# wzjin2017/fhe-fed

Hardware: AMD Instinct MI355X
Metric: ciphertexts aggregated/sec (+ encode+enc / dec+decode ms), N clients, ring 2^15 L=4 (higher is better)
Workload: dtype u64; 1 GPU; cfg3: 16 learners/GPU x ResNet-18 (11689512 params -> 714 cts of 16384 slots), ring 2^15, L=4 towers; ring_dim=32768, towers=4, learners_total=16, cts_per_learner=714, parallelism=dp1 (one GPU, no collective), layout=arena

## Files before the change

fhe-fed_amd/csrc/dev_common.h:

```cpp
#pragma once

#include <hip/hip_runtime.h>

#include "shelfi_internal.h"

namespace shelfi {

typedef uint32_t u32x4 __attribute__((ext_vector_type(4)));

__device__ __forceinline__ uint64_t addmod(uint64_t a, uint64_t b, uint64_t q) {
  uint64_t s = a + b;
  return s >= q ? s - q : s;
}
__device__ __forceinline__ uint64_t submod(uint64_t a, uint64_t b, uint64_t q) {
  return a >= b ? a - b : a + q - b;
}
__device__ __forceinline__ uint64_t shoup_mul(uint64_t x, uint64_t w, uint64_t wp, uint64_t q) {
  uint64_t hi = __umul64hi(x, wp);
  uint64_t r = x * w - hi * q;
  return r >= q ? r - q : r;
}
__device__ __forceinline__ uint64_t red64(uint64_t x, uint64_t q, uint64_t one_sh) {
  uint64_t hi = __umul64hi(x, one_sh);
  uint64_t r = x - hi * q;
// ... 11 lines not shown
  const uint32_t c1 = x1 * w0 + x0 * w1, c2 = h1 * n0 + h0 * n1;
  uint32_t hi;
  asm("v_add3_u32 %0, %1, %2, %3" : "=v"(hi) : "v"((uint32_t)(lo >> 32)), "v"(c1), "v"(c2));
  return ((uint64_t)hi << 32) | (uint32_t)lo;
}
__device__ __forceinline__ uint64_t shoup_lazy_add(uint64_t x, uint64_t w, uint64_t wp, uint64_t q, uint64_t a) {
  const uint64_t h = umulhi_approx(x, wp), nq = (uint64_t)0 - q;
  const uint32_t x0 = (uint32_t)x, x1 = (uint32_t)(x >> 32), w0 = (uint32_t)w, w1 = (uint32_t)(w >> 32);
  const uint32_t h0 = (uint32_t)h, h1 = (uint32_t)(h >> 32), n0 = (uint32_t)nq, n1 = (uint32_t)(nq >> 32);
  const uint64_t lo = (uint64_t)h0 * n0 + ((uint64_t)x0 * w0 + a);
  const uint32_t c1 = x1 * w0 + x0 * w1, c2 = h1 * n0 + h0 * n1;
  uint32_t hi;
  asm("v_add3_u32 %0, %1, %2, %3" : "=v"(hi) : "v"((uint32_t)(lo >> 32)), "v"(c1), "v"(c2));
  return ((uint64_t)hi << 32) | (uint32_t)lo;
}
__device__ __forceinline__ uint64_t shoup_lazy_sub(uint64_t x, uint64_t w, uint64_t wp, uint64_t q) {
  return x * w - umulhi_approx(x, wp) * q;
}
__device__ __forceinline__ uint64_t sub4q_if_ge(uint64_t X, uint64_t q) {
  uint64_t d;
  const bool borrow = __builtin_sub_overflow(X, q << 2, &d);
  return borrow ? X : d;
}
__device__ __forceinline__ void ct_bfly(uint64_t& X, uint64_t& Y, uint64_t W, uint64_t Wp,
                                        uint64_t q) {
  const uint64_t x = sub4q_if_ge(X, q);
  const uint64_t t = shoup_lazy(Y, W, Wp, q);
  X = x + t;
  Y = x + (q << 2) - t;
}
__device__ __forceinline__ void gs_bfly(uint64_t& X, uint64_t& Y, uint64_t W, uint64_t Wp,
                                        uint64_t q) {
  const uint64_t s = X + Y;
  const uint64_t d = X + (q << 2) - Y;
  X = sub4q_if_ge(s, q);
  Y = shoup_lazy_sub(d, W, Wp, q);
}
__device__ __forceinline__ uint32_t bfi32(uint32_t m, uint32_t a, uint32_t b) {
  uint32_t r;
  asm("v_bfi_b32 %0, %1, %2, %3" : "=v"(r) : "v"(m), "v"(a), "v"(b));
  return r;
}
__device__ __forceinline__ uint64_t csub_neg(uint64_t x, uint64_t negc) {
  const uint64_t d = x + negc;
  const uint32_t m = (uint32_t)((int32_t)(uint32_t)(d >> 32) >> 31);
  const uint32_t lo = bfi32(m, (uint32_t)x, (uint32_t)d);
  const uint32_t hi = bfi32(m, (uint32_t)(x >> 32), (uint32_t)(d >> 32));
  return ((uint64_t)hi << 32) | lo;
}
__device__ __forceinline__ uint64_t red_any(uint64_t x, const TowerConst& c) {
  const uint32_t k = __umulhi((uint32_t)(x >> 32), c.red_r) >> c.red_sh;
  const uint64_t r = x + (uint64_t)k * (uint32_t)c.nq + ((uint64_t)(k * (uint32_t)(c.nq >> 32)) << 32);
  return csub_neg(r, c.nq);
}
constexpr uint64_t kNoRedQ = 1ull << 57;
constexpr bool fwd_red_at(int s) {
  int B = 1;
  for (int i = 0; i < s; ++i) B = (B + 4 > 16 ? 8 : B) + 4;
  return B + 4 > 16;
}
constexpr int fwd_bound(int S) {
  int B = 1;
  for (int i = 0; i < S; ++i) B = (B + 4 > 16 ? 8 : B) + 4;
  return B;
}
template <bool RED>
__device__ __forceinline__ void ct_bfly_s(uint64_t& X, uint64_t& Y, uint64_t W, uint64_t Wp,
                                          uint64_t q, uint64_t n8q) {
  const uint64_t x = RED ? csub_neg(X, n8q) : X;
  const uint64_t s = shoup_lazy_add(Y, W, Wp, q, x);
  Y = (x << 1) + (q << 2) - s;
  X = s;
}

__device__ __forceinline__ void gs_bfly_s(uint64_t& X, uint64_t& Y, uint64_t W, uint64_t Wp,
                                          uint64_t q, uint64_t n4q) {
  const uint64_t x = X, y = Y;
  X = csub_neg(x + y, n4q);
  Y = shoup_lazy(x + (q << 2) - y, W, Wp, q);
}
template <bool B8>
__device__ __forceinline__ void gs_bfly_b(uint64_t& X, uint64_t& Y, uint64_t W, uint64_t Wp, uint64_t q,
                                          uint64_t n8q) {
  const uint64_t x = X, y = Y;
  X = B8 ? csub_neg(x + y, n8q) : x + y;
  Y = shoup_lazy(x + (q << (B8 ? 3 : 2)) - y, W, Wp, q);
}
template <bool IN8>
__device__ constexpr bool gs_in8(int v, int a) {
  return v == 0 ? IN8 : ((a >> (v - 1)) & 1) == 0;
}
__device__ __forceinline__ uint64_t canon8(uint64_t x, uint64_t q) {
  x = x >= 4 * q ? x - 4 * q : x;
  x = x >= 2 * q ? x - 2 * q : x;
  return x >= q ? x - q : x;
}
__device__ __forceinline__ uint64_t canon4(uint64_t x, uint64_t q) {
  x = x >= 2 * q ? x - 2 * q : x;
  return x >= q ? x - q : x;
}

__device__ __forceinline__ uint64_t mulmod_generic(uint64_t a, uint64_t b, const TowerConst& c) {
  uint64_t hi = __umul64hi(a, b), lo = a * b;
  return addmod(shoup_mul(hi, c.r64, c.r64_shoup, c.q), red64(lo, c.q, c.one_shoup), c.q);
}
__device__ __forceinline__ uint64_t mod_signed_dev(int64_t v, const TowerConst& c) {
// ... 425 lines not shown
```

fhe-fed_amd/csrc/keyswitch.hip:

```cpp
#include <hip/hip_runtime.h>

#include <algorithm>

#include "dev_common.h"
#include "shelfi_internal.h"

namespace shelfi {

typedef unsigned __int128 du128;

#define NTT_DISPATCH_KS(LOGRV, KERNEL, ...)                                               \
  switch (LOGRV) {                                                                       \
    case 1: hipLaunchKernelGGL(KERNEL<1>, __VA_ARGS__); break;                           \
    case 2: hipLaunchKernelGGL(KERNEL<2>, __VA_ARGS__); break;                           \
    case 3: hipLaunchKernelGGL(KERNEL<3>, __VA_ARGS__); break;                           \
    case 4: hipLaunchKernelGGL(KERNEL<4>, __VA_ARGS__); break;                           \
    case 5: hipLaunchKernelGGL(KERNEL<5>, __VA_ARGS__); break;                           \
    case 6: hipLaunchKernelGGL(KERNEL<6>, __VA_ARGS__); break;                           \
    default: throw Error{SHELFI_ERR_ARG, "EvalMult: unsupported ring dimension"};        \
  }

__device__ __forceinline__ uint64_t red128(du128 acc, const TowerConst& c) {
  const uint64_t hi = (uint64_t)(acc >> 64), lo = (uint64_t)acc;
  return addmod(shoup_mul(hi, c.r64, c.r64_shoup, c.q), red64(lo, c.q, c.one_shoup), c.q);
}
__device__ __forceinline__ du128 mul128(uint64_t a, uint64_t b) { return (du128)a * b; }

__device__ __forceinline__ void digit_span(const KsArgs& a, uint32_t j, uint32_t& s, uint32_t& cnt) {
  s = j * a.alpha;
  cnt = min(a.alpha, a.Ll - s);
}
__device__ __forceinline__ uint64_t ext_base(const KsArgs& a, uint32_t j, uint64_t K) {
  uint64_t base = 0;
  for (uint32_t i = 0; i < j; ++i) {
    uint32_t s, cnt;
    digit_span(a, i, s, cnt);
    base += (uint64_t)(a.T - cnt) * K;
  }
  return base << a.logN;
}

__global__ __launch_bounds__(256) void ks_tensor_intt_kernel(const uint64_t* x, const uint64_t* y, uint32_t Ll,
                                                             uint32_t logN, uint32_t blkLog,
                                                             const uint64_t* __restrict__ itw,
                                                             const uint64_t* __restrict__ itwp,
                                                             const TowerConst* __restrict__ tq, uint64_t* out,
                                                             uint64_t* __restrict__ d2e,
                                                             uint64_t* __restrict__ d2c) {
  extern __shared__ __attribute__((aligned(16))) uint64_t sm[];
  const uint32_t N = 1u << logN, blk = 1u << blkLog, sh = logN - blkLog;
  const uint64_t row = blockIdx.x >> sh;
  const uint32_t b = blockIdx.x & ((1u << sh) - 1);
  const uint64_t k = row / Ll;
  const uint32_t t = (uint32_t)(row % Ll);
  const TowerConst c = tq[t];
  const uint64_t q = c.q;
  const uint64_t off = ((uint64_t)t << logN) + ((uint64_t)b << blkLog);
  const uint64_t i0 = ((k * 2 * Ll) << logN) + off, i1 = (((k * 2 + 1) * Ll) << logN) + off;
  const uint64_t id = (row << logN) + ((uint64_t)b << blkLog);
  const ulonglong2* A0 = reinterpret_cast<const ulonglong2*>(x + i0);
  const ulonglong2* A1 = reinterpret_cast<const ulonglong2*>(x + i1);
  const ulonglong2* B0 = reinterpret_cast<const ulonglong2*>(y + i0);
  const ulonglong2* B1 = reinterpret_cast<const ulonglong2*>(y + i1);
  ulonglong2* O0 = reinterpret_cast<ulonglong2*>(out + i0);
  ulonglong2* O1 = reinterpret_cast<ulonglong2*>(out + i1);
  ulonglong2* E2 = reinterpret_cast<ulonglong2*>(d2e + id);
  for (uint32_t p = threadIdx.x; p < blk / 2; p += 256) {
    const ulonglong2 a0 = A0[p], a1 = A1[p], b0 = B0[p], b1 = B1[p];
    const ulonglong2 r0 = make_ulonglong2(mulmod_generic(a0.x, b0.x, c), mulmod_generic(a0.y, b0.y, c));
    const ulonglong2 r1 =
        make_ulonglong2(addmod(mulmod_generic(a0.x, b1.x, c), mulmod_generic(a1.x, b0.x, c), q),
                        addmod(mulmod_generic(a0.y, b1.y, c), mulmod_generic(a1.y, b0.y, c), q));
    const ulonglong2 r2 = make_ulonglong2(mulmod_generic(a1.x, b1.x, c), mulmod_generic(a1.y, b1.y, c));
    O0[p] = r0;
    O1[p] = r1;
    E2[p] = r2;
    lds_put2(sm, p, r2);
  }
  __syncthreads();
  ks_intt_block_out(sm, blkLog, b, logN, itw + (uint64_t)t * N, itwp + (uint64_t)t * N, c, d2c + id);
}

__global__ __launch_bounds__(256) void modup_kernel(const uint64_t* __restrict__ c, uint64_t K,
                                                    KsArgs a, uint64_t* __restrict__ ext) {
  const uint32_t N = 1u << a.logN, bpr = N >> 8;
  const uint64_t row = blockIdx.x / bpr;
  const uint32_t n = (blockIdx.x % bpr) * 256 + threadIdx.x;
  const uint32_t j = (uint32_t)(row / K);
  const uint64_t k = row % K;
  uint32_t s, cnt;
  digit_span(a, j, s, cnt);
  uint64_t yv[kMaxTowers];
  for (uint32_t i = 0; i < cnt; ++i) {
    const TowerConst ci = a.tq[s + i];
    yv[i] = shoup_mul(c[((k * a.Ll + s + i) << a.logN) + n], a.mu_inv[j * a.alpha + i],
                      a.mu_inv_sh[j * a.alpha + i], ci.q);
  }
  const uint32_t Tf = a.T - cnt;
  uint64_t* __restrict__ o = ext + ext_base(a, j, K) + ((k * Tf) << a.logN) + n;
  for (uint32_t u = 0; u < Tf; ++u) {
    const uint32_t t = u < s ? u : u + cnt;
    du128 acc = 0;
    const uint64_t* __restrict__ h = a.mu_hat + (uint64_t)j * a.alpha * a.T + t;
    for (uint32_t i = 0; i < cnt; ++i) acc += mul128(yv[i], h[(uint64_t)i * a.T]);
    o[(uint64_t)u << a.logN] = red128(acc, a.te[t]);
  }
}

template <int LOGR>
__global__ __launch_bounds__(256) void modup_cols_kernel(const uint64_t* __restrict__ c, uint64_t K, KsArgs a,
                                                         const uint64_t* __restrict__ tw,
                                                         const uint64_t* __restrict__ twp,
                                                         uint64_t* __restrict__ ext) {
  constexpr int R = 1 << LOGR;
  const uint32_t N = 1u << a.logN, BLK = N >> LOGR, bpp = BLK / 256;
  const uint64_t row = blockIdx.x / bpp;
  const uint32_t col = (blockIdx.x % bpp) * 256 + threadIdx.x;
  const uint32_t j = (uint32_t)(row / K);
  const uint64_t k = row % K;
  uint32_t s, cnt;
  digit_span(a, j, s, cnt);
  uint64_t y[2][R];
#pragma unroll
  for (int i = 0; i < 2; ++i) {
    if ((uint32_t)i < cnt) {
      const TowerConst ci = a.tq[s + i];
      const uint64_t w = a.mu_inv[j * a.alpha + i], wp = a.mu_inv_sh[j * a.alpha + i];
      const uint64_t* __restrict__ src = c + ((k * a.Ll + s + i) << a.logN) + col;
#pragma unroll
      for (int r = 0; r < R; ++r) y[i][r] = shoup_mul(src[(uint64_t)r * BLK], w, wp, ci.q);
    }
  }
  const uint32_t Tf = a.T - cnt;
  uint64_t* __restrict__ o = ext + ext_base(a, j, K) + ((k * Tf) << a.logN) + col;
  for (uint32_t u = 0; u < Tf; ++u) {
    const uint32_t t = u < s ? u : u + cnt;
    const TowerConst ct = a.te[t];
    const uint64_t h0 = a.mu_hat[(uint64_t)j * a.alpha * a.T + t];
    const uint64_t h1 = cnt > 1 ? a.mu_hat[((uint64_t)j * a.alpha + 1) * a.T + t] : 0;
    uint64_t x[R];
#pragma unroll
    for (int r = 0; r < R; ++r) {
      du128 acc = mul128(y[0][r], h0);
      if (cnt > 1) acc += mul128(y[1][r], h1);
      x[r] = red128(acc, ct);
    }
    const uint64_t* __restrict__ w = tw + (uint64_t)t * N;
    const uint64_t* __restrict__ wp = twp + (uint64_t)t * N;
#pragma unroll
    for (int st = 0; st < LOGR; ++st) {
      const int m = 1 << st, tr = R >> (st + 1);
#pragma unroll
      for (int i = 0; i < m; ++i) {
        const uint64_t W = w[m + i], Wp = wp[m + i];
#pragma unroll
        for (int jj = 0; jj < tr; ++jj) {
          const int r0 = 2 * i * tr + jj, r1 = r0 + tr;
          ct_bfly(x[r0], x[r1], W, Wp, ct.q);
        }
      }
    }
    uint64_t* __restrict__ ou = o + ((uint64_t)u << a.logN);
#pragma unroll
    for (int r = 0; r < R; ++r) ou[(uint64_t)r * BLK] = x[r];
  }
}

template <int LOGR>
__global__ __launch_bounds__(256) void moddown_cols_kernel(const uint64_t* __restrict__ accP, KsArgs a,
                                                           const uint64_t* __restrict__ tw,
                                                           const uint64_t* __restrict__ twp,
                                                           uint64_t* __restrict__ z) {
  constexpr int R = 1 << LOGR;
  const uint32_t N = 1u << a.logN, BLK = N >> LOGR, bpp = BLK / 256;
  const uint64_t row = blockIdx.x / bpp;
  const uint32_t col = (blockIdx.x % bpp) * 256 + threadIdx.x;
  uint64_t y[2][R];
#pragma unroll
  for (int m = 0; m < 2; ++m) {
    if ((uint32_t)m < a.kP) {
      const TowerConst cp = a.te[a.Ll + m];
      const uint64_t* __restrict__ src = accP + ((row * a.kP + m) << a.logN) + col;
#pragma unroll
      for (int r = 0; r < R; ++r) y[m][r] = shoup_mul(src[(uint64_t)r * BLK], a.md_inv[m], a.md_inv_sh[m], cp.q);
    }
  }
  for (uint32_t t = 0; t < a.Ll; ++t) {
    const TowerConst ct = a.tq[t];
    const uint64_t h0 = a.md_hat[t], h1 = a.kP > 1 ? a.md_hat[(uint64_t)a.Ll + t] : 0;
    uint64_t x[R];
#pragma unroll
    for (int r = 0; r < R; ++r) {
      du128 acc = mul128(y[0][r], h0);
      if (a.kP > 1) acc += mul128(y[1][r], h1);
      x[r] = red128(acc, ct);
    }
    const uint64_t* __restrict__ w = tw + (uint64_t)t * N;
    const uint64_t* __restrict__ wp = twp + (uint64_t)t * N;
#pragma unroll
    for (int st = 0; st < LOGR; ++st) {
      const int m = 1 << st, tr = R >> (st + 1);
#pragma unroll
      for (int i = 0; i < m; ++i) {
        const uint64_t W = w[m + i], Wp = wp[m + i];
#pragma unroll
        for (int jj = 0; jj < tr; ++jj) {
          const int r0 = 2 * i * tr + jj, r1 = r0 + tr;
          ct_bfly(x[r0], x[r1], W, Wp, ct.q);
        }
      }
    }
    uint64_t* __restrict__ ot = z + ((row * a.Ll + t) << a.logN) + col;
#pragma unroll
    for (int r = 0; r < R; ++r) ot[(uint64_t)r * BLK] = x[r];
  }
}

__global__ __launch_bounds__(256) void ks_inner_blocks_kernel(const uint64_t* __restrict__ d2e,
                                                              const uint64_t* __restrict__ ext, uint64_t K,
                                                              KsArgs a, uint32_t blkLog,
                                                              const uint64_t* __restrict__ tw,
                                                              const uint64_t* __restrict__ twp,
                                                              const uint64_t* __restrict__ evk,
                                                              const uint64_t* __restrict__ evk_sh,
                                                              uint64_t* __restrict__ accQ,
                                                              uint64_t* __restrict__ accP) {
  extern __shared__ __attribute__((aligned(16))) uint64_t sm[];
  const uint32_t N = 1u << a.logN, blk = 1u << blkLog, sh = a.logN - blkLog;
  const uint64_t row = blockIdx.x >> sh;
  const uint32_t b = blockIdx.x & ((1u << sh) - 1);
  const uint64_t k = row / a.T;
  const uint32_t t = (uint32_t)(row % a.T);
  const TowerConst c = a.te[t];
  const uint64_t q = c.q;
  const uint32_t TF = a.Lfull + a.kP;
  const uint32_t tk = t < a.Ll ? t : a.Lfull + (t - a.Ll);
  const uint64_t boff = (uint64_t)b << blkLog;
  uint32_t own_mask = 0;
  for (uint32_t j = 0; j < a.dn; ++j) {
    uint32_t s, cnt;
    digit_span(a, j, s, cnt);
    if (t >= s && t < s + cnt) {
      own_mask |= 1u << j;
      continue;
    }
    const uint32_t u = t < s ? t : t - cnt;
    const ulonglong2* src = reinterpret_cast<const ulonglong2*>(
        ext + ext_base(a, j, K) + ((k * (a.T - cnt) + u) << a.logN) + boff);
    for (uint32_t p = threadIdx.x; p < blk / 2; p += 256) lds_put2(sm + ((uint64_t)j << blkLog), p, src[p]);
  }
  __syncthreads();
  for (uint32_t j = 0; j < a.dn; ++j)
    if (!(own_mask & (1u << j)))
      ntt_fwd_block_stages(sm + ((uint64_t)j << blkLog), blkLog, b, a.logN, tw + (uint64_t)t * N,
                           twp + (uint64_t)t * N, q);
  const ulonglong2* own_src = reinterpret_cast<const ulonglong2*>(d2e + ((k * a.Ll + t) << a.logN) + boff);
  ulonglong2 *o0, *o1;
  if (t < a.Ll) {
    o0 = reinterpret_cast<ulonglong2*>(accQ + ((((k * 2 + 0) * a.Ll + t)) << a.logN) + boff);
    o1 = reinterpret_cast<ulonglong2*>(accQ + ((((k * 2 + 1) * a.Ll + t)) << a.logN) + boff);
  } else {
    const uint32_t m = t - a.Ll;
    o0 = reinterpret_cast<ulonglong2*>(accP + ((((k * 2 + 0) * a.kP + m)) << a.logN) + boff);
    o1 = reinterpret_cast<ulonglong2*>(accP + ((((k * 2 + 1) * a.kP + m)) << a.logN) + boff);
// ... 8 lines not shown
        v = lds_get2(sm + ((uint64_t)j << blkLog), p);
        v = make_ulonglong2(canon8(v.x, q), canon8(v.y, q));
      }
      const uint64_t kb = ((((uint64_t)j * TF + tk)) << a.logN) + boff + 2ull * p;
      const uint64_t ka = ((((uint64_t)(a.dnFull + j) * TF + tk)) << a.logN) + boff + 2ull * p;
      const ulonglong2 bv = *reinterpret_cast<const ulonglong2*>(evk + kb);
      const ulonglong2 bs = *reinterpret_cast<const ulonglong2*>(evk_sh + kb);
      const ulonglong2 av = *reinterpret_cast<const ulonglong2*>(evk + ka);
      const ulonglong2 as = *reinterpret_cast<const ulonglong2*>(evk_sh + ka);
      u0.x = addmod(u0.x, shoup_mul(v.x, bv.x, bs.x, q), q);
      u0.y = addmod(u0.y, shoup_mul(v.y, bv.y, bs.y, q), q);
      u1.x = addmod(u1.x, shoup_mul(v.x, av.x, as.x, q), q);
      u1.y = addmod(u1.y, shoup_mul(v.y, av.y, as.y, q), q);
    }
    o0[p] = u0;
    o1[p] = u1;
  }
}

template <int BL, int K1, int K2, int K3, int K4>
__global__ __launch_bounds__(256) void ks_inner_blocks_ct(const uint64_t* __restrict__ d2e,
                                                          const uint64_t* __restrict__ ext, uint64_t K, KsArgs a,
                                                          const ulonglong2* __restrict__ twb,
                                                          const uint64_t* __restrict__ evk,
                                                          const uint64_t* __restrict__ evk_sh,
                                                          uint64_t* __restrict__ accQ, uint64_t* __restrict__ accP) {
  extern __shared__ __attribute__((aligned(16))) uint64_t sm[];
  constexpr uint32_t SL = lpad_size(BL);
  const uint32_t sh = a.logN - BL;
  const uint64_t row = blockIdx.x >> sh;
  const uint32_t b = blockIdx.x & ((1u << sh) - 1);
  const uint64_t k = row / a.T;
  const uint32_t t = (uint32_t)(row % a.T);
  const TowerConst& c = a.te[t];
  const uint64_t q = c.q;
  const uint32_t TF = a.Lfull + a.kP;
  const uint32_t tk = t < a.Ll ? t : a.Lfull + (t - a.Ll);
  const uint64_t boff = (uint64_t)b << BL;
  const ulonglong2* __restrict__ tb = twb + ((uint64_t)t << a.logN) + boff;
  uint32_t own_mask = 0;
  for (uint32_t j = 0; j < a.dn; ++j) {
    uint32_t s, cnt;
    digit_span(a, j, s, cnt);
    if (t >= s && t < s + cnt) {
      own_mask |= 1u << j;
      continue;
    }
    const uint32_t u = t < s ? t : t - cnt;
    uint64_t* slot = sm + (uint64_t)j * SL;
    fwd_block_pass_ct<BL, K1, K2, K3, K4>(ext + ext_base(a, j, K) + ((k * (a.T - cnt) + u) << a.logN) + boff, tb,
                                          q, c.n8q, slot, [&](uint32_t j0, auto& x) {
                                            const uint32_t pj0 = lpad(j0);
#pragma unroll
                                            for (int m = 0; m < (1 << K4); ++m) slot[pj0 + m] = red_any(x[m], c);
                                          });
  }
  __syncthreads();
  const ulonglong2* own_src = reinterpret_cast<const ulonglong2*>(d2e + ((k * a.Ll + t) << a.logN) + boff);
  ulonglong2 *o0, *o1;
  if (t < a.Ll) {
    o0 = reinterpret_cast<ulonglong2*>(accQ + ((((k * 2 + 0) * a.Ll + t)) << a.logN) + boff);
    o1 = reinterpret_cast<ulonglong2*>(accQ + ((((k * 2 + 1) * a.Ll + t)) << a.logN) + boff);
  } else {
    const uint32_t m = t - a.Ll;
    o0 = reinterpret_cast<ulonglong2*>(accP + ((((k * 2 + 0) * a.kP + m)) << a.logN) + boff);
    o1 = reinterpret_cast<ulonglong2*>(accP + ((((k * 2 + 1) * a.kP + m)) << a.logN) + boff);
  }
  for (uint32_t p = threadIdx.x; p < (1u << BL) / 2; p += 256) {
    ulonglong2 u0 = make_ulonglong2(0, 0), u1 = make_ulonglong2(0, 0);
    for (uint32_t j = 0; j < a.dn; ++j) {
      const ulonglong2 v = (own_mask & (1u << j))
                               ? own_src[p]
                               : *reinterpret_cast<const ulonglong2*>(sm + (uint64_t)j * SL + lpad(2 * p));
      const uint64_t kb = ((((uint64_t)j * TF + tk)) << a.logN) + boff + 2ull * p;
      const uint64_t ka = ((((uint64_t)(a.dnFull + j) * TF + tk)) << a.logN) + boff + 2ull * p;
      const ulonglong2 bv = *reinterpret_cast<const ulonglong2*>(evk + kb);
      const ulonglong2 bs = *reinterpret_cast<const ulonglong2*>(evk_sh + kb);
      const ulonglong2 av = *reinterpret_cast<const ulonglong2*>(evk + ka);
      const ulonglong2 as = *reinterpret_cast<const ulonglong2*>(evk_sh + ka);
      u0.x = addmod(u0.x, shoup_mul(v.x, bv.x, bs.x, q), q);
      u0.y = addmod(u0.y, shoup_mul(v.y, bv.y, bs.y, q), q);
      u1.x = addmod(u1.x, shoup_mul(v.x, av.x, as.x, q), q);
      u1.y = addmod(u1.y, shoup_mul(v.y, av.y, as.y, q), q);
    }
    o0[p] = u0;
    o1[p] = u1;
  }
}

__global__ __launch_bounds__(256) void moddown_kernel(const uint64_t* __restrict__ accP, KsArgs a,
                                                      uint64_t* __restrict__ z) {
  const uint32_t N = 1u << a.logN, bpr = N >> 8;
  const uint64_t row = blockIdx.x / bpr;
  const uint32_t n = (blockIdx.x % bpr) * 256 + threadIdx.x;
  uint64_t yv[kMaxTowers];
  for (uint32_t m = 0; m < a.kP; ++m) {
    const TowerConst cp = a.te[a.Ll + m];
    yv[m] = shoup_mul(accP[(row * a.kP + m) * N + n], a.md_inv[m], a.md_inv_sh[m], cp.q);
  }
  for (uint32_t t = 0; t < a.Ll; ++t) {
    du128 acc = 0;
    for (uint32_t m = 0; m < a.kP; ++m) acc += mul128(yv[m], a.md_hat[(uint64_t)m * a.Ll + t]);
    z[(row * a.Ll + t) * N + n] = red128(acc, a.tq[t]);
  }
}

__global__ __launch_bounds__(256) void ks_finish_blocks_kernel(const uint64_t* __restrict__ z,
                                                               const uint64_t* __restrict__ accQ, KsArgs a,
                                                               uint32_t blkLog, const uint64_t* __restrict__ tw,
                                                               const uint64_t* __restrict__ twp,
                                                               uint64_t* __restrict__ out) {
  extern __shared__ __attribute__((aligned(16))) uint64_t sm[];
  const uint32_t N = 1u << a.logN, blk = 1u << blkLog, sh = a.logN - blkLog;
  const uint64_t row = blockIdx.x >> sh;
  const uint32_t b = blockIdx.x & ((1u << sh) - 1);
  const uint32_t t = (uint32_t)(row % a.Ll);
  const TowerConst c = a.tq[t];
  const uint64_t q = c.q, pinv = a.pinv[t], pinv_sh = a.pinv_sh[t];
  const uint64_t off = (row << a.logN) + ((uint64_t)b << blkLog);
  const ulonglong2* Z = reinterpret_cast<const ulonglong2*>(z + off);
  for (uint32_t p = threadIdx.x; p < blk / 2; p += 256) lds_put2(sm, p, Z[p]);
  __syncthreads();
  ntt_fwd_block_stages(sm, blkLog, b, a.logN, tw + (uint64_t)t * N, twp + (uint64_t)t * N, q);
  const ulonglong2* AQ = reinterpret_cast<const ulonglong2*>(accQ + off);
  ulonglong2* O = reinterpret_cast<ulonglong2*>(out + off);
  for (uint32_t p = threadIdx.x; p < blk / 2; p += 256) {
    const ulonglong2 v = lds_get2(sm, p), aq = AQ[p], o = O[p];
    const uint64_t dx = submod(aq.x, canon8(v.x, q), q), dy = submod(aq.y, canon8(v.y, q), q);
    O[p] = make_ulonglong2(addmod(o.x, shoup_mul(dx, pinv, pinv_sh, q), q),
                           addmod(o.y, shoup_mul(dy, pinv, pinv_sh, q), q));
  }
}

template <int BL, int K1, int K2, int K3, int K4>
__global__ __launch_bounds__(256) void ks_finish_blocks_ct(const uint64_t* __restrict__ z,
                                                           const uint64_t* __restrict__ accQ, KsArgs a,
                                                           const ulonglong2* __restrict__ twb,
                                                           uint64_t* __restrict__ out) {
  __shared__ __attribute__((aligned(16))) uint64_t sm[lpad_size(BL)];
  const uint32_t sh = a.logN - BL;
  const uint64_t row = blockIdx.x >> sh;
  const uint32_t b = blockIdx.x & ((1u << sh) - 1);
  const uint32_t t = (uint32_t)(row % a.Ll);
  const TowerConst& c = a.tq[t];
  const uint64_t q = c.q, pinv = a.pinv[t], pinv_sh = a.pinv_sh[t];
  const uint64_t off = (row << a.logN) + ((uint64_t)b << BL);
  const ulonglong2* __restrict__ tb = twb + ((uint64_t)t << a.logN) + ((uint64_t)b << BL);
  fwd_block_pass_ct<BL, K1, K2, K3, K4>(z + off, tb, q, c.n8q, sm, [&](uint32_t j0, auto& x) {
#pragma unroll
    for (int m = 0; m < (1 << K4); m += 2) {
      const ulonglong2 aq = *reinterpret_cast<const ulonglong2*>(accQ + off + j0 + m);
      ulonglong2* O = reinterpret_cast<ulonglong2*>(out + off + j0 + m);
      const ulonglong2 o = *O;
      const uint64_t dx = submod(aq.x, red_any(x[m], c), q), dy = submod(aq.y, red_any(x[m + 1], c), q);
      *O = make_ulonglong2(addmod(o.x, shoup_mul(dx, pinv, pinv_sh, q), q),
                           addmod(o.y, shoup_mul(dy, pinv, pinv_sh, q), q));
    }
  });
}

size_t ks_scratch_bytes(uint32_t Ll, uint32_t kP, uint32_t dn, uint32_t alpha, uint32_t N, uint64_t K) {
  const uint64_t T = Ll + kP;
  uint64_t ext = 0;
  for (uint32_t j = 0; j < dn; ++j) ext += T - std::min(alpha, Ll - j * alpha);
  return K * (uint64_t)N * 8 * (2ull * Ll + ext + 2ull * Ll + 2ull * kP + 2ull * Ll) + 64;
}

KsScratch ks_scratch_layout(const KsArgs& a, uint64_t K, void* scratch) {
  const uint64_t KN = K << a.logN;
  KsScratch k;
  k.d2e = reinterpret_cast<uint64_t*>(scratch);
  k.d2c = k.d2e + KN * a.Ll;
  k.ext = k.d2c + KN * a.Ll;
  uint64_t next = 0;
  for (uint32_t j = 0; j < a.dn; ++j) next += a.T - std::min(a.alpha, a.Ll - j * a.alpha);
  k.accQ = k.ext + KN * next;
  k.accP = k.accQ + KN * 2 * a.Ll;
  k.z = k.accP + KN * 2 * a.kP;
  return k;
}

void launch_eval_mult(const KsArgs& a, const DeviceTables& dtq, const DeviceTables& dte,
                      const DeviceTables* dtf, const uint64_t* evk, const uint64_t* evk_sh, const uint64_t* x,
                      const uint64_t* y, uint64_t K, uint64_t* out, void* scratch, hipStream_t s) {
  if (!K) return;
  const uint32_t blkLog = ntt_block_log(a.logN), sh = a.logN - blkLog;
  const KsScratch ks = ks_scratch_layout(a, K, scratch);
  const uint64_t blocks = (K * a.Ll) << sh;
  if (blocks > 0x7FFFFFFFull) throw Error{SHELFI_ERR_ARG, "EvalMult batch too large"};
  hipLaunchKernelGGL(ks_tensor_intt_kernel, dim3((uint32_t)blocks), dim3(256), sizeof(uint64_t) << blkLog, s, x, y,
                     a.Ll, a.logN, blkLog, dtq.ipsi_rev, dtq.ipsi_rev_sh, a.tq, out, ks.d2e, ks.d2c);
  SHELFI_HIP(hipGetLastError());
  launch_key_switch(a, dtq, dte, dtf, evk, evk_sh, K, out, scratch, s);
}

void launch_key_switch(const KsArgs& a, const DeviceTables& dtq, const DeviceTables& dte, const DeviceTables* dtf,
                       const uint64_t* evk, const uint64_t* evk_sh, uint64_t K, uint64_t* out, void* scratch,
                       hipStream_t s) {
  if (!K) return;
  const uint32_t N = 1u << a.logN, bpr = N >> 8;
  const uint32_t blkLog = ntt_block_log(a.logN), sh = a.logN - blkLog;
  const size_t lds = sizeof(uint64_t) << blkLog;
  const uint64_t KN = K * N;
  const KsScratch ks = ks_scratch_layout(a, K, scratch);
  uint64_t *d2e = ks.d2e, *d2c = ks.d2c, *ext = ks.ext, *accQ = ks.accQ, *accP = ks.accP, *z = ks.z;
  auto grid = [&](uint64_t rows, uint32_t per_row) {
    const uint64_t b = rows * per_row;
    if (b > 0x7FFFFFFFull) throw Error{SHELFI_ERR_ARG, "key switch batch too large"};
    return dim3((uint32_t)b);
  };
  const uint32_t nb = 1u << sh;
  launch_ntt_cols(d2c, K * a.Ll, a.Ll, a.logN, true, dtq, s);
  const int logR = (int)sh;
  const bool fuse_cols = logR > 0 && logR <= 4 && a.alpha <= 2 && a.kP <= 2;
  if (fuse_cols) {
    const uint64_t rows = (uint64_t)a.dn * K, per = (N >> logR) / 256;
    NTT_DISPATCH_KS(logR, modup_cols_kernel, grid(rows, (uint32_t)per), dim3(256), 0, s, d2c, K, a, dte.psi_rev,
                    dte.psi_rev_sh, ext);
  } else {
    hipLaunchKernelGGL(modup_kernel, grid((uint64_t)a.dn * K, bpr), dim3(256), 0, s, d2c, K, a, ext);
    uint64_t* e = ext;
    for (uint32_t j = 0; j < a.dn && logR > 0; ++j) {
      const uint32_t Tf = a.T - std::min(a.alpha, a.Ll - j * a.alpha);
      launch_ntt_cols(e, K * Tf, Tf, a.logN, false, dtf[j], s);
      e += KN * Tf;
    }
  }
  SHELFI_HIP(hipGetLastError());
  if (sh > 0 && blkLog == 11 && dte.red_ok) {
    hipLaunchKernelGGL((ks_inner_blocks_ct<11, 3, 3, 3, 2>), grid(K * a.T, nb), dim3(256),
                       sizeof(uint64_t) * lpad_size(11) * a.dn, s, d2e, ext, K, a, dte.tw_fwd_blk, evk, evk_sh, accQ,
                       accP);
  } else {
    if (lds * a.dn > 65536)
      SHELFI_HIP(hipFuncSetAttribute(reinterpret_cast<const void*>(&ks_inner_blocks_kernel),
                                     hipFuncAttributeMaxDynamicSharedMemorySize, (int)(lds * a.dn)));
    hipLaunchKernelGGL(ks_inner_blocks_kernel, grid(K * a.T, nb), dim3(256), lds * a.dn, s, d2e, ext, K, a, blkLog,
                       dte.psi_rev, dte.psi_rev_sh, evk, evk_sh, accQ, accP);
  }
  SHELFI_HIP(hipGetLastError());
  launch_ntt(accP, K * 2 * a.kP, a.kP, a.logN, true, tower_view(dte, a.Ll, N), s);
  if (fuse_cols) {
    NTT_DISPATCH_KS(logR, moddown_cols_kernel, grid(K * 2, (uint32_t)((N >> logR) / 256)), dim3(256), 0, s, accP, a,
                    dtq.psi_rev, dtq.psi_rev_sh, z);
  } else {
    hipLaunchKernelGGL(moddown_kernel, grid(K * 2, bpr), dim3(256), 0, s, accP, a, z);
    SHELFI_HIP(hipGetLastError());
    launch_ntt_cols(z, K * 2 * a.Ll, a.Ll, a.logN, false, dtq, s);
  }
  SHELFI_HIP(hipGetLastError());
  if (sh > 0 && blkLog == 11 && dtq.red_ok)
    hipLaunchKernelGGL((ks_finish_blocks_ct<11, 3, 3, 3, 2>), grid(K * 2 * a.Ll, nb), dim3(256), 0, s, z, accQ, a,
                       dtq.tw_fwd_blk, out);
  else if (sh > 0 && blkLog == 12 && dtq.red_ok)
    hipLaunchKernelGGL((ks_finish_blocks_ct<12, 3, 3, 3, 3>), grid(K * 2 * a.Ll, nb), dim3(256), 0, s, z, accQ, a,
                       dtq.tw_fwd_blk, out);
  else
    hipLaunchKernelGGL(ks_finish_blocks_kernel, grid(K * 2 * a.Ll, nb), dim3(256), lds, s, z, accQ, a, blkLog,
                       dtq.psi_rev, dtq.psi_rev_sh, out);
  SHELFI_HIP(hipGetLastError());
}

__global__ __launch_bounds__(256) void rescale_lift_kernel(const uint64_t* __restrict__ last, uint32_t Lo,
                                                           uint32_t logN, uint64_t ql,
                                                           const TowerConst* __restrict__ tq,
                                                           uint64_t* __restrict__ v) {
  const uint32_t N = 1u << logN, bpr = N >> 8;
  const uint64_t row = blockIdx.x / bpr;
  const uint32_t n = (blockIdx.x % bpr) * 256 + threadIdx.x;
  const uint32_t t = (uint32_t)(row % Lo);
  const TowerConst c = tq[t];
  const uint64_t x = last[(row / Lo) * N + n];
  uint64_t r;
  if (x > (ql >> 1)) {
    const uint64_t m = red64(ql - x, c.q, c.one_shoup);
    r = m ? c.q - m : 0;
  } else {
    r = red64(x, c.q, c.one_shoup);
  }
  v[row * N + n] = r;
}

__global__ __launch_bounds__(256) void rescale_finish_blocks_kernel(const uint64_t* __restrict__ in,
                                                                    const uint64_t* __restrict__ v, uint32_t Lo,
                                                                    uint32_t logN, uint32_t blkLog,
                                                                    const uint64_t* __restrict__ tw,
                                                                    const uint64_t* __restrict__ twp,
                                                                    const TowerConst* __restrict__ tq,
                                                                    RescaleConst rc, uint64_t* __restrict__ out) {
  extern __shared__ __attribute__((aligned(16))) uint64_t sm[];
  const uint32_t N = 1u << logN, blk = 1u << blkLog, sh = logN - blkLog;
  const uint64_t row = blockIdx.x >> sh;
  const uint32_t b = blockIdx.x & ((1u << sh) - 1);
  const uint64_t kp = row / Lo;
  const uint32_t t = (uint32_t)(row % Lo);
  const uint64_t q = tq[t].q, w = rc.qlinv[t], wp = rc.qlinv_sh[t];
  const uint64_t boff = (uint64_t)b << blkLog;
  const ulonglong2* V = reinterpret_cast<const ulonglong2*>(v + (row << logN) + boff);
  for (uint32_t p = threadIdx.x; p < blk / 2; p += 256) lds_put2(sm, p, V[p]);
  __syncthreads();
  ntt_fwd_block_stages(sm, blkLog, b, logN, tw + (uint64_t)t * N, twp + (uint64_t)t * N, q);
  const ulonglong2* X = reinterpret_cast<const ulonglong2*>(in + ((kp * (Lo + 1) + t) << logN) + boff);
  ulonglong2* O = reinterpret_cast<ulonglong2*>(out + (row << logN) + boff);
  for (uint32_t p = threadIdx.x; p < blk / 2; p += 256) {
    const ulonglong2 y = lds_get2(sm, p), x = X[p];
    O[p] = make_ulonglong2(shoup_mul(submod(x.x, canon8(y.x, q), q), w, wp, q),
                           shoup_mul(submod(x.y, canon8(y.y, q), q), w, wp, q));
  }
}

size_t rescale_scratch_bytes(uint32_t Ll, uint32_t N, uint64_t K) {
  return K * 2ull * N * 8 * (1 + (uint64_t)(Ll - 1)) + 64;
}

template <int BL, int K1, int K2, int K3, int K4>
__global__ __launch_bounds__(256) void rescale_finish_blocks_ct(const uint64_t* __restrict__ in,
                                                                const uint64_t* __restrict__ v, uint32_t Lo,
                                                                uint32_t logN, const ulonglong2* __restrict__ twb,
                                                                const TowerConst* __restrict__ tq, RescaleConst rc,
                                                                uint64_t* __restrict__ out) {
  __shared__ __attribute__((aligned(16))) uint64_t sm[lpad_size(BL)];
  const uint32_t sh = logN - BL;
  const uint64_t row = blockIdx.x >> sh;
  const uint32_t b = blockIdx.x & ((1u << sh) - 1);
  const uint64_t kp = row / Lo;
  const uint32_t t = (uint32_t)(row % Lo);
  const TowerConst& c = tq[t];
  const uint64_t q = c.q, w = rc.qlinv[t], wp = rc.qlinv_sh[t];
  const uint64_t boff = (uint64_t)b << BL;
  const ulonglong2* __restrict__ tb = twb + ((uint64_t)t << logN) + boff;
  const uint64_t* __restrict__ X = in + ((kp * (Lo + 1) + t) << logN) + boff;
  uint64_t* __restrict__ O = out + (row << logN) + boff;
  fwd_block_pass_ct<BL, K1, K2, K3, K4>(v + (row << logN) + boff, tb, q, c.n8q, sm, [&](uint32_t j0, auto& y) {
#pragma unroll
    for (int m = 0; m < (1 << K4); m += 2) {
      const ulonglong2 x = *reinterpret_cast<const ulonglong2*>(X + j0 + m);
      *reinterpret_cast<ulonglong2*>(O + j0 + m) =
          make_ulonglong2(shoup_mul(submod(x.x, red_any(y[m], c), q), w, wp, q),
                          shoup_mul(submod(x.y, red_any(y[m + 1], c), q), w, wp, q));
    }
  });
}

void launch_rescale(const DeviceTables& dt, uint32_t Ll, uint32_t logN, const RescaleConst& rc,
                    const uint64_t* in, uint64_t K, uint64_t* out, void* scratch, hipStream_t s) {
  if (!K) return;
  const uint32_t N = 1u << logN, bpr = N >> 8, Lo = Ll - 1;
  uint64_t* last = reinterpret_cast<uint64_t*>(scratch);
  uint64_t* v = last + K * 2 * N;
  SHELFI_HIP(hipMemcpy2DAsync(last, (size_t)N * 8, in + (uint64_t)Lo * N, (size_t)Ll * N * 8, (size_t)N * 8,
                              K * 2, hipMemcpyDeviceToDevice, s));
  launch_ntt(last, K * 2, 1, logN, true, tower_view(dt, Lo, N), s);
  const uint64_t rows = K * 2 * Lo;
  if (rows * bpr > 0x7FFFFFFFull) throw Error{SHELFI_ERR_ARG, "ModReduce batch too large"};
  hipLaunchKernelGGL(rescale_lift_kernel, dim3((uint32_t)(rows * bpr)), dim3(256), 0, s, last, Lo, logN, rc.ql,
                     dt.tc, v);
  SHELFI_HIP(hipGetLastError());
  launch_ntt_cols(v, rows, Lo, logN, false, dt, s);
  const uint32_t blkLog = ntt_block_log(logN);
  const dim3 nbf((uint32_t)(rows << (logN - blkLog)));
  if (logN > blkLog && blkLog == 11 && dt.red_ok)
    hipLaunchKernelGGL((rescale_finish_blocks_ct<11, 3, 3, 3, 2>), nbf, dim3(256), 0, s, in, v, Lo, logN,
                       dt.tw_fwd_blk, dt.tc, rc, out);
  else if (logN > blkLog && blkLog == 12 && dt.red_ok)
    hipLaunchKernelGGL((rescale_finish_blocks_ct<12, 3, 3, 3, 3>), nbf, dim3(256), 0, s, in, v, Lo, logN,
                       dt.tw_fwd_blk, dt.tc, rc, out);
  else
    hipLaunchKernelGGL(rescale_finish_blocks_kernel, nbf, dim3(256), sizeof(uint64_t) << blkLog, s, in, v, Lo,
                       logN, blkLog, dt.psi_rev, dt.psi_rev_sh, dt.tc, rc, out);
  SHELFI_HIP(hipGetLastError());
}

__global__ __launch_bounds__(256) void evk_sample_kernel(uint32_t logN, uint32_t T0,
                                                         const TowerConst* __restrict__ te,
                                                         const uint64_t* __restrict__ cdt, int T, Key8 key,
                                                         uint64_t nonce_base, uint32_t j,
                                                         uint64_t* __restrict__ e_out,
                                                         uint64_t* __restrict__ a_out) {
  const uint32_t N = 1u << logN;
  const uint32_t gid = blockIdx.x * 256 + threadIdx.x;
  if (gid >= (N >> 3)) return;
  const uint32_t j0 = gid * 8;
  const uint64_t nonce = nonce_base | ((uint64_t)j << 16);
  uint64_t re[8];
  chacha20_block(key, j0 >> 3, nonce, re);
  int64_t ev[8];
#pragma unroll
  for (int u = 0; u < 8; ++u) ev[u] = gauss_sample(re[u], cdt, T);
  for (uint32_t t = 0; t < T0; ++t) {
    const TowerConst c = te[t];
    uint64_t ra[16];
    chacha20_block(key, j0 >> 2, nonce | (1 + t), ra);
// ... 91 lines not shown
```

Measured before the change: 3.447 million client-ciphertexts/s.

## Use lazy modular reduction across keyswitch, modup/moddown column NTTs and rescale

Replaces the full modular reductions in the keyswitch tensor, the modup/moddown fused column NTT stages, the inner-product accumulation, the finish kernels and rescale with lazy reductions. These use a 2^60 split for 128-bit products, lazy Shoup butterflies with bounded growth, and a periodic red_any. The goal is fewer conditional subtractions and multiplies in these ALU-bound kernels. The code also adds sched_barrier hints to order the tensor products. Correctness now depends on the tracked bounds (values below 12q) and on the red_ok flags, and extra template variants increase code size.

```diff
diff --git a/fhe-fed_amd/csrc/dev_common.h b/fhe-fed_amd/csrc/dev_common.h
--- a/fhe-fed_amd/csrc/dev_common.h
+++ b/fhe-fed_amd/csrc/dev_common.h
@@ -87,6 +87,10 @@
   const uint32_t k = __umulhi((uint32_t)(x >> 32), c.red_r) >> c.red_sh;
   const uint64_t r = x + (uint64_t)k * (uint32_t)c.nq + ((uint64_t)(k * (uint32_t)(c.nq >> 32)) << 32);
   return csub_neg(r, c.nq);
+}
+__device__ __forceinline__ uint64_t red128_any(unsigned __int128 acc, const TowerConst& c) {
+  const uint64_t h = (uint64_t)(acc >> 60), l = (uint64_t)acc & ((1ull << 60) - 1);
+  return red_any(shoup_lazy_add(h, c.r60, c.r60_shoup, c.q, l), c);
 }
 constexpr uint64_t kNoRedQ = 1ull << 57;
 constexpr bool fwd_red_at(int s) {
diff --git a/fhe-fed_amd/csrc/keyswitch.hip b/fhe-fed_amd/csrc/keyswitch.hip
--- a/fhe-fed_amd/csrc/keyswitch.hip
+++ b/fhe-fed_amd/csrc/keyswitch.hip
@@ -9,14 +9,12 @@
 
 typedef unsigned __int128 du128;
 
-#define NTT_DISPATCH_KS(LOGRV, KERNEL, ...)                                               \
+#define KS_DISPATCH_COLS(LOGRV, KERNEL, LAZY, ...)                                        \
   switch (LOGRV) {                                                                       \
-    case 1: hipLaunchKernelGGL(KERNEL<1>, __VA_ARGS__); break;                           \
-    case 2: hipLaunchKernelGGL(KERNEL<2>, __VA_ARGS__); break;                           \
-    case 3: hipLaunchKernelGGL(KERNEL<3>, __VA_ARGS__); break;                           \
-    case 4: hipLaunchKernelGGL(KERNEL<4>, __VA_ARGS__); break;                           \
-    case 5: hipLaunchKernelGGL(KERNEL<5>, __VA_ARGS__); break;                           \
-    case 6: hipLaunchKernelGGL(KERNEL<6>, __VA_ARGS__); break;                           \
+    case 1: hipLaunchKernelGGL((KERNEL<1, LAZY>), __VA_ARGS__); break;                   \
+    case 2: hipLaunchKernelGGL((KERNEL<2, LAZY>), __VA_ARGS__); break;                   \
+    case 3: hipLaunchKernelGGL((KERNEL<3, LAZY>), __VA_ARGS__); break;                   \
+    case 4: hipLaunchKernelGGL((KERNEL<4, LAZY>), __VA_ARGS__); break;                   \
     default: throw Error{SHELFI_ERR_ARG, "EvalMult: unsupported ring dimension"};        \
   }
 
@@ -40,7 +38,8 @@
   return base << a.logN;
 }
 
-__global__ __launch_bounds__(256) void ks_tensor_intt_kernel(const uint64_t* x, const uint64_t* y, uint32_t Ll,
+template <bool RED>
+__global__ __launch_bounds__(256) void ks_tensor_intt_kernel(const uint64_t* x, const uint64_t* y, const uint32_t Ll,
                                                              uint32_t logN, uint32_t blkLog,
                                                              const uint64_t* __restrict__ itw,
                                                              const uint64_t* __restrict__ itwp,
@@ -53,7 +52,7 @@
   const uint32_t b = blockIdx.x & ((1u << sh) - 1);
   const uint64_t k = row / Ll;
   const uint32_t t = (uint32_t)(row % Ll);
-  const TowerConst c = tq[t];
+  const TowerConst& c = tq[t];
   const uint64_t q = c.q;
   const uint64_t off = ((uint64_t)t << logN) + ((uint64_t)b << blkLog);
   const uint64_t i0 = ((k * 2 * Ll) << logN) + off, i1 = (((k * 2 + 1) * Ll) << logN) + off;
@@ -65,17 +64,36 @@
   ulonglong2* O0 = reinterpret_cast<ulonglong2*>(out + i0);
   ulonglong2* O1 = reinterpret_cast<ulonglong2*>(out + i1);
   ulonglong2* E2 = reinterpret_cast<ulonglong2*>(d2e + id);
-  for (uint32_t p = threadIdx.x; p < blk / 2; p += 256) {
-    const ulonglong2 a0 = A0[p], a1 = A1[p], b0 = B0[p], b1 = B1[p];
-    const ulonglong2 r0 = make_ulonglong2(mulmod_generic(a0.x, b0.x, c), mulmod_generic(a0.y, b0.y, c));
-    const ulonglong2 r1 =
-        make_ulonglong2(addmod(mulmod_generic(a0.x, b1.x, c), mulmod_generic(a1.x, b0.x, c), q),
-                        addmod(mulmod_generic(a0.y, b1.y, c), mulmod_generic(a1.y, b0.y, c), q));
-    const ulonglong2 r2 = make_ulonglong2(mulmod_generic(a1.x, b1.x, c), mulmod_generic(a1.y, b1.y, c));
-    O0[p] = r0;
-    O1[p] = r1;
-    E2[p] = r2;
-    lds_put2(sm, p, r2);
+  if (RED) {
+    for (uint32_t p = threadIdx.x; p < blk / 2; p += 256) {
+      const ulonglong2 a0 = A0[p], a1 = A1[p], b0 = B0[p], b1 = B1[p];
+      __builtin_amdgcn_sched_barrier(0);
+      const ulonglong2 r1 = make_ulonglong2(red128_any(mul128(a0.x, b1.x) + mul128(a1.x, b0.x), c),
+                                            red128_any(mul128(a0.y, b1.y) + mul128(a1.y, b0.y), c));
+      O1[p] = r1;
+      __builtin_amdgcn_sched_barrier(0);
+      const ulonglong2 r0 = make_ulonglong2(red128_any(mul128(a0.x, b0.x), c), red128_any(mul128(a0.y, b0.y), c));
+      O0[p] = r0;
+      __builtin_amdgcn_sched_barrier(0);
+      const ulonglong2 r2 = make_ulonglong2(red128_any(mul128(a1.x, b1.x), c), red128_any(mul128(a1.y, b1.y), c));
+      E2[p] = r2;
+      lds_put2(sm, p, r2);
+    }
+  } else {
+    for (uint32_t p = threadIdx.x; p < blk / 2; p += 256) {
+      const ulonglong2 a0 = A0[p], a1 = A1[p], b0 = B0[p], b1 = B1[p];
+      const ulonglong2 r1 =
+          make_ulonglong2(addmod(mulmod_generic(a0.x, b1.x, c), mulmod_generic(a1.x, b0.x, c), q),
+                          addmod(mulmod_generic(a0.y, b1.y, c), mulmod_generic(a1.y, b0.y, c), q));
+      O1[p] = r1;
+      __builtin_amdgcn_sched_barrier(0);
+      const ulonglong2 r0 = make_ulonglong2(mulmod_generic(a0.x, b0.x, c), mulmod_generic(a0.y, b0.y, c));
+      O0[p] = r0;
+      __builtin_amdgcn_sched_barrier(0);
+      const ulonglong2 r2 = make_ulonglong2(mulmod_generic(a1.x, b1.x, c), mulmod_generic(a1.y, b1.y, c));
+      E2[p] = r2;
+      lds_put2(sm, p, r2);
+    }
   }
   __syncthreads();
   ks_intt_block_out(sm, blkLog, b, logN, itw + (uint64_t)t * N, itwp + (uint64_t)t * N, c, d2c + id);
@@ -107,7 +125,37 @@
   }
 }
 
-template <int LOGR>
+constexpr bool cols_red_at(int s, int S) { return fwd_red_at(s) || (s == S - 1 && fwd_bound(s) > 8); }
+constexpr int cols_bound(int S) {
+  return S == 0 ? 1 : (cols_red_at(S - 1, S) ? 8 : fwd_bound(S - 1)) + 4;
+}
+static_assert(cols_bound(1) <= 12 && cols_bound(2) <= 12 && cols_bound(3) <= 12 && cols_bound(4) <= 12,
+              "the fused column stages hand fwd_block_pass_ct values below 12q");
+template <int LOGR, bool LAZY>
+__device__ __forceinline__ void ks_col_stages(uint64_t (&x)[1 << LOGR], const uint64_t* __restrict__ w,
+                                              const uint64_t* __restrict__ wp, const TowerConst& ct) {
+  constexpr int R = 1 << LOGR;
+#pragma unroll
+  for (int st = 0; st < LOGR; ++st) {
+    const int m = 1 << st, tr = R >> (st + 1);
+#pragma unroll
+    for (int i = 0; i < m; ++i) {
+      const uint64_t W = w[m + i], Wp = wp[m + i];
+#pragma unroll
+      for (int jj = 0; jj < tr; ++jj) {
+        const int r0 = 2 * i * tr + jj, r1 = r0 + tr;
+        if (!LAZY)
+          ct_bfly(x[r0], x[r1], W, Wp, ct.q);
+        else if (cols_red_at(st, LOGR))
+          ct_bfly_s<true>(x[r0], x[r1], W, Wp, ct.q, ct.n8q);
+        else
+          ct_bfly_s<false>(x[r0], x[r1], W, Wp, ct.q, ct.n8q);
+      }
+    }
+  }
+}
+
+template <int LOGR, bool LAZY>
 __global__ __launch_bounds__(256) void modup_cols_kernel(const uint64_t* __restrict__ c, uint64_t K, KsArgs a,
                                                          const uint64_t* __restrict__ tw,
                                                          const uint64_t* __restrict__ twp,
@@ -141,32 +189,27 @@
     uint64_t x[R];
 #pragma unroll
     for (int r = 0; r < R; ++r) {
-      du128 acc = mul128(y[0][r], h0);
-      if (cnt > 1) acc += mul128(y[1][r], h1);
-      x[r] = red128(acc, ct);
-    }
-    const uint64_t* __restrict__ w = tw + (uint64_t)t * N;
-    const uint64_t* __restrict__ wp = twp + (uint64_t)t * N;
-#pragma unroll
-    for (int st = 0; st < LOGR; ++st) {
-      const int m = 1 << st, tr = R >> (st + 1);
-#pragma unroll
-      for (int i = 0; i < m; ++i) {
-        const uint64_t W = w[m + i], Wp = wp[m + i];
-#pragma unroll
-        for (int jj = 0; jj < tr; ++jj) {
-          const int r0 = 2 * i * tr + jj, r1 = r0 + tr;
-          ct_bfly(x[r0], x[r1], W, Wp, ct.q);
-        }
+      if (LAZY) {
+        du128 acc;
+        if (cnt > 1)
+          acc = mul128(y[0][r], h0) + mul128(y[1][r], h1);
+        else
+          acc = mul128(y[0][r], h0);
+        x[r] = red128_any(acc, ct);
+      } else {
+        du128 acc = mul128(y[0][r], h0);
+        if (cnt > 1) acc += mul128(y[1][r], h1);
+        x[r] = red128(acc, ct);
       }
     }
+    ks_col_stages<LOGR, LAZY>(x, tw + (uint64_t)t * N, twp + (uint64_t)t * N, ct);
     uint64_t* __restrict__ ou = o + ((uint64_t)u << a.logN);
 #pragma unroll
     for (int r = 0; r < R; ++r) ou[(uint64_t)r * BLK] = x[r];
   }
 }
 
-template <int LOGR>
+template <int LOGR, bool LAZY>
 __global__ __launch_bounds__(256) void moddown_cols_kernel(const uint64_t* __restrict__ accP, KsArgs a,
                                                            const uint64_t* __restrict__ tw,
                                                            const uint64_t* __restrict__ twp,
@@ -191,25 +234,20 @@
     uint64_t x[R];
 #pragma unroll
     for (int r = 0; r < R; ++r) {
-      du128 acc = mul128(y[0][r], h0);
-      if (a.kP > 1) acc += mul128(y[1][r], h1);
-      x[r] = red128(acc, ct);
-    }
-    const uint64_t* __restrict__ w = tw + (uint64_t)t * N;
-    const uint64_t* __restrict__ wp = twp + (uint64_t)t * N;
-#pragma unroll
-    for (int st = 0; st < LOGR; ++st) {
-      const int m = 1 << st, tr = R >> (st + 1);
-#pragma unroll
-      for (int i = 0; i < m; ++i) {
-        const uint64_t W = w[m + i], Wp = wp[m + i];
-#pragma unroll
-        for (int jj = 0; jj < tr; ++jj) {
-          const int r0 = 2 * i * tr + jj, r1 = r0 + tr;
-          ct_bfly(x[r0], x[r1], W, Wp, ct.q);
-        }
+      if (LAZY) {
+        du128 acc;
+        if (a.kP > 1)
+          acc = mul128(y[0][r], h0) + mul128(y[1][r], h1);
+        else
+          acc = mul128(y[0][r], h0);
+        x[r] = red128_any(acc, ct);
+      } else {
+        du128 acc = mul128(y[0][r], h0);
+        if (a.kP > 1) acc += mul128(y[1][r], h1);
+        x[r] = red128(acc, ct);
       }
     }
+    ks_col_stages<LOGR, LAZY>(x, tw + (uint64_t)t * N, twp + (uint64_t)t * N, ct);
     uint64_t* __restrict__ ot = z + ((row * a.Ll + t) << a.logN) + col;
 #pragma unroll
     for (int r = 0; r < R; ++r) ot[(uint64_t)r * BLK] = x[r];
@@ -324,7 +362,7 @@
                                           q, c.n8q, slot, [&](uint32_t j0, auto& x) {
                                             const uint32_t pj0 = lpad(j0);
 #pragma unroll
-                                            for (int m = 0; m < (1 << K4); ++m) slot[pj0 + m] = red_any(x[m], c);
+                                            for (int m = 0; m < (1 << K4); ++m) slot[pj0 + m] = x[m];
                                           });
   }
   __syncthreads();
@@ -341,6 +379,10 @@
   for (uint32_t p = threadIdx.x; p < (1u << BL) / 2; p += 256) {
     ulonglong2 u0 = make_ulonglong2(0, 0), u1 = make_ulonglong2(0, 0);
     for (uint32_t j = 0; j < a.dn; ++j) {
+      if (j && j % 3 == 0) {
+        u0 = make_ulonglong2(red_any(u0.x, c), red_any(u0.y, c));
+        u1 = make_ulonglong2(red_any(u1.x, c), red_any(u1.y, c));
+      }
       const ulonglong2 v = (own_mask & (1u << j))
                                ? own_src[p]
                                : *reinterpret_cast<const ulonglong2*>(sm + (uint64_t)j * SL + lpad(2 * p));
@@ -350,13 +392,13 @@
       const ulonglong2 bs = *reinterpret_cast<const ulonglong2*>(evk_sh + kb);
       const ulonglong2 av = *reinterpret_cast<const ulonglong2*>(evk + ka);
       const ulonglong2 as = *reinterpret_cast<const ulonglong2*>(evk_sh + ka);
-      u0.x = addmod(u0.x, shoup_mul(v.x, bv.x, bs.x, q), q);
-      u0.y = addmod(u0.y, shoup_mul(v.y, bv.y, bs.y, q), q);
-      u1.x = addmod(u1.x, shoup_mul(v.x, av.x, as.x, q), q);
-      u1.y = addmod(u1.y, shoup_mul(v.y, av.y, as.y, q), q);
-    }
-    o0[p] = u0;
-    o1[p] = u1;
+      u0.x = shoup_lazy_add(v.x, bv.x, bs.x, q, u0.x);
+      u0.y = shoup_lazy_add(v.y, bv.y, bs.y, q, u0.y);
+      u1.x = shoup_lazy_add(v.x, av.x, as.x, q, u1.x);
+      u1.y = shoup_lazy_add(v.y, av.y, as.y, q, u1.y);
+    }
+    o0[p] = make_ulonglong2(red_any(u0.x, c), red_any(u0.y, c));
+    o1[p] = make_ulonglong2(red_any(u1.x, c), red_any(u1.y, c));
   }
 }
 
@@ -418,15 +460,16 @@
   const uint64_t q = c.q, pinv = a.pinv[t], pinv_sh = a.pinv_sh[t];
   const uint64_t off = (row << a.logN) + ((uint64_t)b << BL);
   const ulonglong2* __restrict__ tb = twb + ((uint64_t)t << a.logN) + ((uint64_t)b << BL);
+  const uint64_t q12 = (q << 3) + (q << 2);
   fwd_block_pass_ct<BL, K1, K2, K3, K4>(z + off, tb, q, c.n8q, sm, [&](uint32_t j0, auto& x) {
 #pragma unroll
     for (int m = 0; m < (1 << K4); m += 2) {
       const ulonglong2 aq = *reinterpret_cast<const ulonglong2*>(accQ + off + j0 + m);
       ulonglong2* O = reinterpret_cast<ulonglong2*>(out + off + j0 + m);
       const ulonglong2 o = *O;
-      const uint64_t dx = submod(aq.x, red_any(x[m], c), q), dy = submod(aq.y, red_any(x[m + 1], c), q);
-      *O = make_ulonglong2(addmod(o.x, shoup_mul(dx, pinv, pinv_sh, q), q),
-                           addmod(o.y, shoup_mul(dy, pinv, pinv_sh, q), q));
+      const uint64_t dx = aq.x + q12 - x[m], dy = aq.y + q12 - x[m + 1];
+      *O = make_ulonglong2(red_any(shoup_lazy_add(dx, pinv, pinv_sh, q, o.x), c),
+                           red_any(shoup_lazy_add(dy, pinv, pinv_sh, q, o.y), c));
     }
   });
 }
@@ -460,8 +503,12 @@
   const KsScratch ks = ks_scratch_layout(a, K, scratch);
   const uint64_t blocks = (K * a.Ll) << sh;
   if (blocks > 0x7FFFFFFFull) throw Error{SHELFI_ERR_ARG, "EvalMult batch too large"};
-  hipLaunchKernelGGL(ks_tensor_intt_kernel, dim3((uint32_t)blocks), dim3(256), sizeof(uint64_t) << blkLog, s, x, y,
-                     a.Ll, a.logN, blkLog, dtq.ipsi_rev, dtq.ipsi_rev_sh, a.tq, out, ks.d2e, ks.d2c);
+  if (dtq.red_ok)
+    hipLaunchKernelGGL(ks_tensor_intt_kernel<true>, dim3((uint32_t)blocks), dim3(256), sizeof(uint64_t) << blkLog, s,
+                       x, y, a.Ll, a.logN, blkLog, dtq.ipsi_rev, dtq.ipsi_rev_sh, a.tq, out, ks.d2e, ks.d2c);
+  else
+    hipLaunchKernelGGL(ks_tensor_intt_kernel<false>, dim3((uint32_t)blocks), dim3(256), sizeof(uint64_t) << blkLog, s,
+                       x, y, a.Ll, a.logN, blkLog, dtq.ipsi_rev, dtq.ipsi_rev_sh, a.tq, out, ks.d2e, ks.d2c);
   SHELFI_HIP(hipGetLastError());
   launch_key_switch(a, dtq, dte, dtf, evk, evk_sh, K, out, scratch, s);
 }
@@ -485,10 +532,17 @@
   launch_ntt_cols(d2c, K * a.Ll, a.Ll, a.logN, true, dtq, s);
   const int logR = (int)sh;
   const bool fuse_cols = logR > 0 && logR <= 4 && a.alpha <= 2 && a.kP <= 2;
+  const bool inner_ct = sh > 0 && blkLog == 11 && dte.red_ok;
+  const bool finish_ct = sh > 0 && (blkLog == 11 || blkLog == 12) && dtq.red_ok;
   if (fuse_cols) {
     const uint64_t rows = (uint64_t)a.dn * K, per = (N >> logR) / 256;
-    NTT_DISPATCH_KS(logR, modup_cols_kernel, grid(rows, (uint32_t)per), dim3(256), 0, s, d2c, K, a, dte.psi_rev,
-                    dte.psi_rev_sh, ext);
+    if (inner_ct) {
+      KS_DISPATCH_COLS(logR, modup_cols_kernel, true, grid(rows, (uint32_t)per), dim3(256), 0, s, d2c, K, a,
+                       dte.psi_rev, dte.psi_rev_sh, ext);
+    } else {
+      KS_DISPATCH_COLS(logR, modup_cols_kernel, false, grid(rows, (uint32_t)per), dim3(256), 0, s, d2c, K, a,
+                       dte.psi_rev, dte.psi_rev_sh, ext);
+    }
   } else {
     hipLaunchKernelGGL(modup_kernel, grid((uint64_t)a.dn * K, bpr), dim3(256), 0, s, d2c, K, a, ext);
     uint64_t* e = ext;
@@ -499,7 +553,7 @@
     }
   }
   SHELFI_HIP(hipGetLastError());
-  if (sh > 0 && blkLog == 11 && dte.red_ok) {
+  if (inner_ct) {
     hipLaunchKernelGGL((ks_inner_blocks_ct<11, 3, 3, 3, 2>), grid(K * a.T, nb), dim3(256),
                        sizeof(uint64_t) * lpad_size(11) * a.dn, s, d2e, ext, K, a, dte.tw_fwd_blk, evk, evk_sh, accQ,
                        accP);
@@ -513,18 +567,23 @@
   SHELFI_HIP(hipGetLastError());
   launch_ntt(accP, K * 2 * a.kP, a.kP, a.logN, true, tower_view(dte, a.Ll, N), s);
   if (fuse_cols) {
-    NTT_DISPATCH_KS(logR, moddown_cols_kernel, grid(K * 2, (uint32_t)((N >> logR) / 256)), dim3(256), 0, s, accP, a,
-                    dtq.psi_rev, dtq.psi_rev_sh, z);
+    if (finish_ct) {
+      KS_DISPATCH_COLS(logR, moddown_cols_kernel, true, grid(K * 2, (uint32_t)((N >> logR) / 256)), dim3(256), 0, s,
+                       accP, a, dtq.psi_rev, dtq.psi_rev_sh, z);
+    } else {
+      KS_DISPATCH_COLS(logR, moddown_cols_kernel, false, grid(K * 2, (uint32_t)((N >> logR) / 256)), dim3(256), 0, s,
+                       accP, a, dtq.psi_rev, dtq.psi_rev_sh, z);
+    }
   } else {
     hipLaunchKernelGGL(moddown_kernel, grid(K * 2, bpr), dim3(256), 0, s, accP, a, z);
     SHELFI_HIP(hipGetLastError());
     launch_ntt_cols(z, K * 2 * a.Ll, a.Ll, a.logN, false, dtq, s);
   }
   SHELFI_HIP(hipGetLastError());
-  if (sh > 0 && blkLog == 11 && dtq.red_ok)
+  if (finish_ct && blkLog == 11)
     hipLaunchKernelGGL((ks_finish_blocks_ct<11, 3, 3, 3, 2>), grid(K * 2 * a.Ll, nb), dim3(256), 0, s, z, accQ, a,
                        dtq.tw_fwd_blk, out);
-  else if (sh > 0 && blkLog == 12 && dtq.red_ok)
+  else if (finish_ct)
     hipLaunchKernelGGL((ks_finish_blocks_ct<12, 3, 3, 3, 3>), grid(K * 2 * a.Ll, nb), dim3(256), 0, s, z, accQ, a,
                        dtq.tw_fwd_blk, out);
   else
@@ -544,7 +603,11 @@
   const TowerConst c = tq[t];
   const uint64_t x = last[(row / Lo) * N + n];
   uint64_t r;
-  if (x > (ql >> 1)) {
+  if (c.red_ok) {
+    const bool neg = x > (ql >> 1);
+    const uint64_t m = red_any(neg ? ql - x : x, c);
+    r = neg ? c.q - m : m;
+  } else if (x > (ql >> 1)) {
     const uint64_t m = red64(ql - x, c.q, c.one_shoup);
     r = m ? c.q - m : 0;
   } else {
@@ -603,13 +666,14 @@
   const ulonglong2* __restrict__ tb = twb + ((uint64_t)t << logN) + boff;
   const uint64_t* __restrict__ X = in + ((kp * (Lo + 1) + t) << logN) + boff;
   uint64_t* __restrict__ O = out + (row << logN) + boff;
+  const uint64_t q12 = (q << 3) + (q << 2);
   fwd_block_pass_ct<BL, K1, K2, K3, K4>(v + (row << logN) + boff, tb, q, c.n8q, sm, [&](uint32_t j0, auto& y) {
 #pragma unroll
     for (int m = 0; m < (1 << K4); m += 2) {
       const ulonglong2 x = *reinterpret_cast<const ulonglong2*>(X + j0 + m);
       *reinterpret_cast<ulonglong2*>(O + j0 + m) =
-          make_ulonglong2(shoup_mul(submod(x.x, red_any(y[m], c), q), w, wp, q),
-                          shoup_mul(submod(x.y, red_any(y[m + 1], c), q), w, wp, q));
+          make_ulonglong2(red_any(shoup_lazy(x.x + q12 - y[m], w, wp, q), c),
+                          red_any(shoup_lazy(x.y + q12 - y[m + 1], w, wp, q), c));
     }
   });
 }
```

Measured after the change: 3.380 million client-ciphertexts/s. 0.981x the previous value.
